# sergcpp/Ray

Hardware: AMD Instinct MI355X
Metric: Msamples/sec (W*H*spp/time) (higher is better)
Workload: dtype f32

## Files before the change

### ray_amd/csrc/rayhip_ctx.hip.h

```cpp
#pragma once

namespace {
thread_local std::string g_err;

int fail(const char *fmt, ...) {
    char buf[1024];
    va_list vl;
    va_start(vl, fmt);
    vsnprintf(buf, sizeof(buf), fmt, vl);
    va_end(vl);
    g_err = buf;
    return 1;
}

#define HIP_TRY(expr)                                                                                                  \
    do {                                                                                                               \
        const hipError_t _e = (expr);                                                                                  \
        if (_e != hipSuccess) {                                                                                        \
            return fail("%s failed: %s (%s:%d)", #expr, hipGetErrorString(_e), __FILE__, __LINE__);                    \
        }                                                                                                              \
    } while (0)

constexpr int MAX_BOUNCE_SLOTS = 130;

// ... 91 lines not shown
    uint32_t cache_path_count = 0;
    DevBuf cache_io;

    int w = 0, h = 0;
    DevBuf px_temp, px_full, px_half, px_raw, px_final, px_base, px_dn, px_req, px_aux_base, px_aux_dn;
    size_t slots_cap = 0;
    DevBuf px_variance, nlm_tm, nlm_var_h, nlm_var;
    DevBuf tonemap_lut;
    DevBuf shard_stage;
    rayhip_update::MeshRefs mesh_refs;
    uint32_t nodes_used = 0, nodes_reserved = 0;
    uint32_t tlas_half = 0;
    int wide = 0;
    uint32_t tex_table[8] = {}, textures_count = 0, tex_flags = 0;
    struct { uint32_t vertices, vtx_indices, tri_materials, materials; } geometry = {};
    bool adaptive_dirty = false;
    int lut_transform = 0, lut_dims = 0;
    PixelBuffers px = {};

    DevBuf ray_planes[2][5], hit_planes[2], shadow_planes[3], deferred_planes[2], point_planes[7], nee_index;
    PointSoA points = {};
    DevBuf pick_plane, record_ray_planes[4];
    RaySoA record_rays = {};
    bool notex_kernels = true;
    bool pick_lds = true;
    bool surface_park = true;
    uint32_t shade_tag = 0;
    uint32_t next_shade_tag() {
        if (++shade_tag == 0u) {
            (void)hipMemsetAsync(pick_plane.p, 0, pick_plane.bytes, stream);
            shade_tag = 1u;
        }
        return shade_tag;
    }
    int shade_split = 29;
    RaySoA rays[2] = {};
    HitSoA hits = {};
    ShadowSoA shadow = {};
    DeferredSoA deferred = {};
    DevBuf counters;
// ... 387 lines not shown
    if (const char *e = getenv("RAYHIP_SORT_KEY")) {
        c->sort_key_mode = std::max(0, std::min(3, atoi(e)));
    }
    if (const char *e = getenv("RAYHIP_SHADE_SPLIT")) {
        c->shade_split = atoi(e) & 31;
        c->shade_form_auto = false;
    }
    if (const char *e = getenv("RAYHIP_NOTEX_KERNELS")) {
        c->notex_kernels = atoi(e) != 0;
    }
    if (const char *e = getenv("RAYHIP_PICK_LDS")) {
        c->pick_lds = atoi(e) != 0;
    }
    if (const char *e = getenv("RAYHIP_SURFACE_PARK")) {
        c->surface_park = atoi(e) != 0;
    }
    {
        const int mode = getenv("RAYHIP_REFILL") != nullptr ? atoi(getenv("RAYHIP_REFILL")) : 3;
        if (mode != 0) {
            int per_cu_refill = 0;
            if (hipOccupancyMaxActiveBlocksPerMultiprocessor(&per_cu_refill, k_trace_closest_refill<8>, WAVE, 0) != hipSuccess || per_cu_refill <= 0) {
                per_cu_refill = per_cu;
            }
            int refill_mult = 16;
            if (const char *e = getenv("RAYHIP_REFILL_MULT")) {
                refill_mult = std::max(1, std::min(64, atoi(e)));
            }
            c->refill_resident = c->props.multiProcessorCount * per_cu_refill;
            {
                int per_cu4 = 0;
// ... 215 lines not shown
```

### ray_amd/csrc/rayhip_render.hip.h

```cpp
#pragma once

static bool pass_fits(const rayhip_ctx *c, const int rect[4], int n) {
    const Layering L = make_layering(c->w, c->h, n);
    const size_t vbytes = size_t(c->w) * size_t(c->h) * size_t(L.cols) * size_t(layer_rows(L)) * 16u;
    return vbytes <= c->px_temp.bytes && (n <= 1 || (vbytes <= c->px_aux_base.bytes && vbytes <= c->px_aux_dn.bytes)) &&
           pass_slots(c, c->w, c->h, rect[2], rect[3], n) + size_t(WAVE) * QUEUE_MAX_STRIPES <= c->slots_cap;
}
static bool rect_inside(const rayhip_ctx *c, const int rect[4]) {
    return rect[0] >= 0 && rect[1] >= 0 && rect[2] > 0 && rect[3] > 0 && rect[0] <= c->w - rect[2] && rect[1] <= c->h - rect[3];
}
static int ensure_pass(rayhip_ctx *c, const int rect[4], int n) {
    if (!rect_inside(c, rect)) {
        return fail("rect outside the frame");
    }
    if (!pass_fits(c, rect, n)) {
        HIP_TRY(hipStreamSynchronize(c->stream));
        if (alloc_frame(c, c->w, c->h, n)) {
            return 1;
        }
    }
    return 0;
}

static void launch_shade(rayhip_ctx *c, const rayhip_camera &cam, int iteration, int bounce, int cur, size_t nslots, uint32_t stripes,
                         int gtrace, int vw, float mix_factor, const Layering &layers, bool plain_ior = false, bool sized = false, int split = -1) {
    ShadeLaunch a;
    a.sc = c->sc;
    a.sp = make_shade_params(cam, iteration, bounce);
    a.sp.plain_ior = plain_ior ? 1u : 0u;
    a.rays_in = c->rays[cur], a.rays_out = c->rays[cur ^ 1];
    a.hits = c->hits, a.shadow = c->shadow, a.deferred = c->deferred, a.points = c->points;
    a.in = c->ray_queue(bounce, nslots, stripes), a.pts = c->point_queue(bounce, nslots, stripes);
    a.out_rays = c->ray_queue(bounce + 1, nslots, stripes), a.out_shadow = c->shadow_queue(bounce, nslots, stripes);
    a.out_deferred = c->deferred_queue(bounce, nslots, stripes), a.nee = c->nee_queue(bounce, nslots, stripes);
    a.out_sky = c->sky_queue(bounce, nslots, stripes), a.sky_index = c->sky_index.as<uint32_t>();
    a.px = c->px, a.layers = layers, a.vw = vw, a.mix_factor = mix_factor;
    a.bounce = bounce, a.grid = gtrace, a.split = split >= 0 ? split : c->shade_split, a.stream = c->stream;
    a.picks = c->pick_plane.as<float4>(), a.record_rays = c->record_rays, a.tag = c->next_shade_tag();
    a.pick_lds = c->pick_lds, a.surface_park = c->surface_park;
    a.no_textures = c->textures_count == 0 && c->notex_kernels;
    if (sized) {
        a.expect[EXPECT_RAYS] = bounce == 0 ? uint32_t(nslots / WAVE + stripes) : c->expect_chunks(bounce, 0, nslots, stripes);
        a.expect[EXPECT_POINTS] = c->expect_chunks(bounce, 3, nslots, stripes), a.expect[EXPECT_LIT] = c->expect_chunks(bounce, 4, nslots, stripes);
        a.expect[EXPECT_DEFERRED] = c->expect_chunks(bounce, 2, nslots, stripes), a.expect[EXPECT_SKY] = c->expect_chunks(bounce, 5, nslots, stripes);
        a.chunks_per_block = c->chunks_per_block;
        a.work = c->next_work(), a.chunks = uint32_t((nslots + WAVE - 1) / WAVE + stripes), a.dyn_mult = c->dyn_mult;
    }
    shade::launch(a);
}

static int render_pass(rayhip_ctx *c, const rayhip_camera *cam, const int rect[4], int iteration, int count_iterations,
                       uint32_t flags, rayhip_stats *stats) {
    if (use_device(c)) {
        return 1;
// ... 346 lines not shown
```

### ray_amd/csrc/rayhip_upload.hip.h

```cpp
#pragma once

static int upload_sky(rayhip_ctx *c, const rayhip_scene_desc *d) {
    c->sky_view = SkyView{};
    if (!(d->env.sky_map_spread_angle > 0.0f) || d->sky_count == 0) {
        return 0;
    }
    if (upload(c, c->sky_desc, d->sky, sizeof(rayhip_sky)) ||
        upload(c, c->sky_transmittance_lut, d->sky_transmittance_lut, size_t(d->sky_transmittance_lut_count) * sizeof(float)) ||
        upload(c, c->sky_multiscatter_lut, d->sky_multiscatter_lut, size_t(d->sky_multiscatter_lut_count) * sizeof(float)) ||
        upload(c, c->sky_dir_lights, d->sky_dir_lights, size_t(d->sky_dir_lights_count) * sizeof(uint32_t)) ||
        upload(c, c->sky_weather, d->sky_weather_tex, d->sky_weather_tex_count) || upload(c, c->sky_noise3d, d->sky_noise3d_tex, d->sky_noise3d_tex_count) ||
        upload(c, c->sky_curl, d->sky_curl_tex, d->sky_curl_tex_count) || upload(c, c->sky_moon, d->sky_moon_tex, d->sky_moon_tex_count) ||
        upload(c, c->sky_cirrus, d->sky_cirrus_tex, d->sky_cirrus_tex_count)) {
        return 1;
    }
    HIP_TRY(hipStreamSynchronize(c->stream));
    SkyView &v = c->sky_view;
    v.desc = c->sky_desc.as<rayhip_sky>();
    v.transmittance_lut = c->sky_transmittance_lut.as<float>(), v.multiscatter_lut = c->sky_multiscatter_lut.as<float>();
    v.dir_lights = c->sky_dir_lights.as<uint32_t>(), v.dir_lights_count = d->sky_dir_lights_count;
    v.weather = c->sky_weather.as<uint8_t>(), v.noise3d = c->sky_noise3d.as<uint8_t>(), v.curl = c->sky_curl.as<uint8_t>();
    v.moon = c->sky_moon.as<uint8_t>(), v.cirrus = c->sky_cirrus.as<uint8_t>();
    return 0;
}
// ... 289 lines not shown
        size_t n_tris = lay.applied ? lay.tris.size() : size_t(d->tris_count);
        rayhip_bvh8::Result b8;
        if (want == 8) {
            b8 = rayhip_bvh8::build(n2, n2_count, mis, d->mesh_instances_count, tlas_root, tris_in, tri_indices_in, uint32_t(n_tris));
            UPLOAD_TRACE(b8.ok ? "bvh8 built" : b8.why_not)
        }
        if (b8.ok && !b8.nodes.empty()) {
            tris_in = b8.tris.data(), tri_indices_in = b8.tri_indices.data(), n_tris = b8.tris.size();
        }
        if (upload(c, c->nodes, n2, size_t(n2_count) * sizeof(rayhip_bvh2_node)) ||
            upload(c, c->tris, tris_in, n_tris * sizeof(rayhip_tri_accel)) ||
            upload(c, c->tri_indices, tri_indices_in, n_tris * sizeof(uint32_t)) ||
            upload(c, c->mesh_instances, mis, size_t(d->mesh_instances_count) * sizeof(rayhip_mesh_instance))) {
            return 1;
        }
        c->tri_pitch = 3;
        if (n_tris && getenv("RAYHIP_TRI_PITCH") && atoi(getenv("RAYHIP_TRI_PITCH")) == 64) {
            DevBuf padded;
            if (padded.alloc(n_tris * 64)) {
                return 1;
            }
            k_pad_tris<<<unsigned((n_tris * 4 + 255) / 256), 256, 0, c->stream>>>(c->tris.as<float4>(), padded.as<float4>(), n_tris);
            HIP_TRY(hipGetLastError());
            HIP_TRY(hipStreamSynchronize(c->stream));
            c->tris.swap(padded);
            padded.release();
            c->tri_pitch = 4;
        }
        size_t wide_bytes = 0;
        if (b8.ok && !b8.nodes.empty()) {
// ... 193 lines not shown
            return 2;
        }
        const uint32_t base = c->nodes_used + c->tlas_half * half;
        c->tlas_half ^= 1u;
        tlas_root = rayhip_update::relocate_top_level(tlas, up, base);
        root_box = tlas.bounds;
        UPLOAD_TRACE("top level built")
        HIP_TRY(hipMemcpyAsync(c->nodes.as<rayhip_bvh2_node>() + base, tlas.nodes.data(), tlas.nodes.size() * sizeof(rayhip_bvh2_node),
                               hipMemcpyHostToDevice, c->stream));
        HIP_TRY(hipStreamSynchronize(c->stream));
    }
    if (upload(c, c->mesh_instances, mis.data(), mis.size() * sizeof(rayhip_mesh_instance)) ||
        (c->wide && upload(c, c->blas_root4, root4.data(), root4.size() * sizeof(uint32_t)))) {
        return 1;
    }
    HIP_TRY(hipStreamSynchronize(c->stream));
    {
        rayhip_scene_desc with_roots = *d;
        if (upload_lights(c, &with_roots) ||
            upload(c, c->env_qtree, d->env_qtree, size_t(d->env_qtree_count) * sizeof(float))) {
            return 1;
        }
    }
    HIP_TRY(hipStreamSynchronize(c->stream));
    if (upload_sky(c, d)) {
        return 1;
    }
    refresh_scene_view(c, d, tlas_root, root_box, uint32_t(live.size()));
    UPLOAD_TRACE("instances updated")
    return 0;
// ... 67 lines not shown
```

### ray_amd/csrc/rt_shade.h

```cpp
#pragma once

#include "rt_sky.h"
#include "shade_lobes.h"

namespace rt {

struct ShadeResult {
    f4 col;
    f3 base_color;
    f4 depth_normal;
    bool emit_secondary, emit_shadow;
    bool defer_sky;
};

RT_HD f3 direct_radiance(const ShadeParams &sp, const Scatter &sct, const f3 throughput) {
    f3 c = sct.direct;
    c *= throughput;
    return clamp_radiance_sum(c, sp.limits[1]);
}
RT_HD float light_pick_random(const SceneView &sc, const ShadeParams &sp, const uint32_t xy, const uint32_t depth) {
    return path_random(sc, sp, xy, depth).get(RAND_DIM_LIGHT_PICK).x;
}
RT_HD LightPick no_light_pick() { return LightPick{0u, 0.0f, 0.0f}; }

RT_HD ShadeResult shade_surface(const SceneView &sc, const ShadeParams &sp, const Hit &hit, const Ray &ray, Ray &new_ray, ShadowRay &sh_r) {
    ShadeResult res;
    res.emit_secondary = res.emit_shadow = false;
    ShadePoint pt;
    SurfaceOut so;
    const bool continues = surface_stage<false>(sc, sp, hit, ray, pt, so);
    res.col = so.radiance;
    res.base_color = so.base_color;
    res.depth_normal = so.normal_depth;
    res.defer_sky = so.deferred_sky;
    if (!continues) {
        return res;
    }
    const LightPick pick = sc.light_cwnodes_count != 0 ? pick_light(sc, pt.P, light_pick_random(sc, sp, ray.xy, ray.depth)) : no_light_pick();
    Scatter sct;
    scatter_stage(sc, sp, ray, pt, pick, sct);
    res.col = mk4(direct_radiance(sp, sct, ray.c), 1.0f);
    res.emit_secondary = sct.has_next, res.emit_shadow = sct.has_shadow;
    new_ray = sct.next, sh_r = sct.shadow;
    return res;
}

}
```

### ray_amd/csrc/shade_kernels.hip

```cpp
#include <hip/hip_runtime.h>

#include <algorithm>
#include <map>
#include <mutex>
#include <utility>

#ifdef RT_PROFILE_SHADE
namespace rt {
__device__ unsigned long long g_prof_shade[64];
}
#define RT_PROF_SHADE_LANES(k)                                                                                          \
    {                                                                                                                   \
        const unsigned long long m_ = __ballot(1);                                                                      \
        if (int(__lane_id()) == __ffsll((long long)m_) - 1) {                                                           \
            atomicAdd(&::rt::g_prof_shade[k], (unsigned long long)__popcll(m_));                                        \
            atomicAdd(&::rt::g_prof_shade[(k) + 1], 1ull);                                                              \
        }                                                                                                               \
    }
#endif

#include "shade_launch.h"

namespace rt {
namespace shade {
// ... 69 lines not shown
            continue;
        }
        const uint32_t i = slot0 + threadIdx.x;
        const bool active = threadIdx.x < n_live;
        bool continues = false, defer = false, sky = false;
        ShadePoint pt;
        SurfaceOut so;
        LightPick pick = no_light_pick();
        if (active) {
            Ray ray = load_ray(rays_in, i, sp.plain_ior == 0u);
            const Hit hit = load_hit(hits, i);
            const uint32_t xy = ray.xy;
            const uint32_t layer = xy_layer(xy, layers);
            const ShadeParams spl = layer_params(sp, layer);
            ray.xy = xy_real(xy, layers, layer);
            continues = surface_stage<true, SKY>(sc, spl, hit, ray, pt, so);
            defer = so.deferred_emitter;
            sky = SKY && so.deferred_sky;
            if (PRIMARY) {
                ShadeResult res;
                res.col = continues ? f4{0.0f, 0.0f, 0.0f, 1.0f} : so.radiance;
                res.base_color = so.base_color, res.depth_normal = so.normal_depth;
                if (layers.count > 1) {
                    write_primary_pixel_layered(res, xy, img_w, px.temp, px.aux_base_layers, px.aux_dn_layers);
                } else {
                    write_primary_pixel(res, xy, img_w, mix_factor, px.temp, px.base_color, px.depth_normals);
                }
            } else if (!continues) {
                ShadeResult res;
                res.col = so.radiance;
                add_secondary_pixel(res, xy, img_w, px.temp);
// ... 156 lines not shown
            }
        }
    }
}

__device__ __forceinline__ uint32_t queue_fill(const RayQueue &q) {
    const uint32_t lane = __lane_id();
    uint32_t n = lane < q.stripes ? q.counts[lane * QUEUE_COUNTER_STRIDE] : 0u;
    for (int m = 32; m >= 1; m >>= 1) {
        n += uint32_t(__shfl_xor(int(n), m));
    }
    return uint32_t(__builtin_amdgcn_readfirstlane(int(n)));
}
__device__ __forceinline__ bool lit_points_are_sparse(const RayQueue &pts, const RayQueue &nee) { return 2u * queue_fill(nee) < queue_fill(pts); }

template <bool NEE, bool CONTINUE, bool INDEXED = false, int MODE = 0>
__global__ void __launch_bounds__(WAVE, (NEE && CONTINUE) ? RT_SCATTER_MIN_WAVES : (NEE ? RT_SCATTER_NEE_MIN_WAVES : RT_SCATTER_CONT_MIN_WAVES)) k_scatter(const SceneView sc, const ShadeParams sp, const RaySoA rays_in,
                                                                       const PointSoA points, const RayQueue in, const RaySoA rays_out,
                                                                       const RayQueue out_rays, const ShadowSoA shadow_out, const RayQueue out_shadow,
                                                                       const PixelBuffers px, const int img_w, const Layering layers,
                                                                       const RayQueue all_points, const RayQueue lit_points) {
    if (MODE != 0 && lit_points_are_sparse(all_points, lit_points) != (MODE == 1)) {
        return;
    }
    const uint32_t n_live_chunks = in.live_chunks();
    ChunkWalk walk(n_live_chunks);
    for (uint32_t c; walk.next(c);) {
        uint32_t stripe, slot0, n_live;
        if (!in.chunk(c, stripe, slot0, n_live)) {
            continue;
        }
        const bool active = threadIdx.x < n_live;
        Scatter sct;
        sct.has_next = sct.has_shadow = false;
        uint32_t xy = 0;
        if (active) {
            uint32_t ray_slot;
            const uint32_t point_slot = INDEXED ? points.nee_index[slot0 + threadIdx.x] : slot0 + threadIdx.x;
            const ShadePoint pt = load_point(points, point_slot, ray_slot);
// ... 1 lines not shown
            Ray ray;
            {
                const float4 d = rays_in.d_cw[ray_slot], cc = rays_in.c_cs[ray_slot];
                const float4 io = sp.plain_ior != 0u ? mkfloat4(-1.0f, -1.0f, -1.0f, -1.0f) : rays_in.ior[ray_slot];
                const uint2 xd = rays_in.xy_depth[ray_slot];
                ray.o = pt.P, ray.pdf = 0.0f;
                ray.d = {d.x, d.y, d.z}, ray.cone_width = d.w;
                ray.c = {cc.x, cc.y, cc.z}, ray.cone_spread = cc.w;
                ray.ior[0] = io.x, ray.ior[1] = io.y, ray.ior[2] = io.z, ray.ior[3] = io.w;
                ray.xy = xd.x, ray.depth = xd.y;
            }
            xy = ray.xy;
            const uint32_t layer = xy_layer(xy, layers);
            const ShadeParams spl = layer_params(sp, layer);
            ray.xy = xy_real(xy, layers, layer);
            scatter_stage<NEE, CONTINUE>(sc, spl, ray, pt, pick, sct);
            sct.next.xy = xy, sct.shadow.xy = xy;
            if (NEE) {
                const f3 col = direct_radiance(spl, sct, ray.c);
                if (col.x != 0.0f || col.y != 0.0f || col.z != 0.0f) {
                    ShadeResult res;
                    res.col = mk4(col, 1.0f);
                    add_secondary_pixel(res, xy, img_w, px.temp);
                }
            }
        }
        if (NEE) {
            const uint32_t sh_slot = out_shadow.alloc(stripe, sct.has_shadow);
            if (sct.has_shadow) {
                store_shadow(shadow_out, sh_slot, sct.shadow);
            }
// ... 109 lines not shown

#ifndef RT_FUSED_NOTEX_MIN_WAVES
#define RT_FUSED_NOTEX_MIN_WAVES 3
#endif
#ifndef RT_FUSED_PARK_MIN_WAVES
#define RT_FUSED_PARK_MIN_WAVES 4
#endif
struct ParkedLane {
    Ray ray;
    float pick[4];
    float pad;
};
constexpr size_t PARK_LDS_BYTES = size_t(WAVE) * sizeof(ParkedLane);
static_assert(sizeof(ParkedLane) % 8u == 4u && PARK_LDS_BYTES <= 10240u, "odd dword stride; at most 10 KB per one-wave block (16 blocks per CU)");
__device__ __forceinline__ void park_fence() { asm volatile("" ::: "memory"); }
template <bool PRIMARY, bool SKY, bool TEX = true, bool PARK = false>
__global__ void __launch_bounds__(WAVE, PARK ? RT_FUSED_PARK_MIN_WAVES : (TEX ? RT_FUSED_MIN_WAVES : RT_FUSED_NOTEX_MIN_WAVES)) k_surface_scatter(const SceneView sc, const ShadeParams sp, const RaySoA rays_in, const HitSoA hits,
                                                                               const RayQueue in, const float4 *__restrict__ picks, const uint32_t tag,
                                                                               const PointSoA records, const RaySoA record_rays, const RayQueue out_records,
                                                                               const RaySoA rays_out, const RayQueue out_rays,
                                                                               const DeferredSoA deferred_out, const RayQueue out_deferred,
                                                                               const PixelBuffers px, const int img_w, const float mix_factor,
                                                                               const Layering layers, uint32_t *__restrict__ sky_index, const RayQueue out_sky) {
    __shared__ ParkedLane s_park[PARK ? WAVE : 1];
    ParkedLane &parked = s_park[PARK ? threadIdx.x : 0u];
    const uint32_t n_live_chunks = in.live_chunks();
    const uint32_t fills = in.fill_counts();
    ChunkWalk walk(n_live_chunks);
    for (uint32_t c; walk.next(c);) {
        uint32_t stripe, slot0, n_live;
        if (!in.chunk(c, fills, stripe, slot0, n_live)) {
            continue;
        }
        const uint32_t i = slot0 + threadIdx.x;
        const bool active = threadIdx.x < n_live;
        bool continues = false, defer = false, sky = false, lit = false;
        ShadePoint pt;
        SurfaceOut so;
        Ray ray_regs;
        Ray &ray = PARK ? parked.ray : ray_regs;
// ... 5 lines not shown
            Ray r = load_ray(rays_in, i, sp.plain_ior == 0u);
            const Hit hit = load_hit(hits, i);
            const float4 pk = picks[i];
            xy = r.xy;
            const uint32_t layer = xy_layer(xy, layers);
            spl = layer_params(sp, layer);
            r.xy = xy_real(xy, layers, layer);
            ahead = vertex_randoms(path_random(sc, spl, r.xy, r.depth));
            if (PARK) {
                parked.ray = r;
                parked.pick[0] = pk.x, parked.pick[1] = pk.y, parked.pick[2] = pk.z, parked.pick[3] = pk.w;
                park_fence();
            } else {
                ray = r, pick = pk;
            }
            continues = surface_stage<true, SKY, TEX>(sc, spl, hit, ray, pt, so, &ahead);
            if (PARK) {
                park_fence();
            }
            defer = so.deferred_emitter;
            sky = SKY && so.deferred_sky;
            if (PRIMARY) {
                ShadeResult res;
                res.col = continues ? f4{0.0f, 0.0f, 0.0f, 1.0f} : so.radiance;
                res.base_color = so.base_color, res.depth_normal = so.normal_depth;
                if (layers.count > 1) {
                    write_primary_pixel_layered(res, xy, img_w, px.temp, px.aux_base_layers, px.aux_dn_layers);
                } else {
                    write_primary_pixel(res, xy, img_w, mix_factor, px.temp, px.base_color, px.depth_normals);
                }
            } else if (!continues) {
// ... 21 lines not shown
            if (sky) {
                sky_index[s_slot] = i;
            }
        }
        if (__any(defer)) {
            const uint32_t d_slot = out_deferred.alloc(stripe, defer);
            if (defer) {
                deferred_out.a[d_slot] = mkfloat4(uint_as_float(i), uint_as_float(so.emitter_triangle), uint_as_float(pt.material), so.emitter_mix_weight);
                deferred_out.b[d_slot] = mkfloat4(pt.base.x, pt.base.y, pt.base.z, 0.0f);
            }
        }
        Scatter sct;
        sct.has_next = sct.has_shadow = false;
        if (continues) {
            ray.o = pt.P, ray.pdf = 0.0f;
            scatter_stage<false, true>(sc, spl, ray, pt, no_light_pick(), sct, &ahead);
            sct.next.xy = xy;
        }
        const uint32_t n_slot = out_rays.alloc(stripe, sct.has_next);
        if (sct.has_next) {
            store_ray(rays_out, n_slot, sct.next, sp.plain_ior == 0u);
        }
    }
}

__global__ void __launch_bounds__(WAVE) k_shade_emissive(const SceneView sc, const ShadeParams sp, const RaySoA rays_in, const HitSoA hits,
                                                        const DeferredSoA deferred, const RayQueue queue, const PixelBuffers px,
                                                        const int img_w) {
    const uint32_t lane = threadIdx.x;
    const uint32_t n_live_chunks = queue.live_chunks();
    ChunkWalk walk(n_live_chunks);
// ... 81 lines not shown
                    const int resident = std::max(1, resident_blocks(reinterpret_cast<const void *>(kernel_wave))) * std::max(1, a.dyn_mult);
                    const uint32_t bound = a.expect[EXPECT_RAYS] != 0u ? a.expect[EXPECT_RAYS] : a.chunks;
                    grid = int(std::max<uint32_t>(1u, std::min<uint32_t>({uint32_t(g), uint32_t(resident), std::max(bound, 1u)})));
                }
                if (lds_nodes != 0u) {
                    kernel<<<(grid + PICK_BLOCK_WAVES - 1) / PICK_BLOCK_WAVES, PICK_BLOCK_WAVES * WAVE, size_t(lds_nodes) * LIGHT_CHILDREN_STRIDE * sizeof(float4), s>>>(
                        a.sc, a.sp, a.rays_in, a.hits, a.in, a.picks, a.tag, a.layers, a.work, lds_nodes);
                } else {
                    kernel_wave<<<grid, WAVE, 0, s>>>(a.sc, a.sp, a.rays_in, a.hits, a.in, a.picks, a.tag, a.layers, a.work, 0u);
                }
            };
            a.work ? go(k_light_pick_first<true, true>, k_light_pick_first<true, false>) : go(k_light_pick_first<false, true>, k_light_pick_first<false, false>);
        }
#define RT_FUSED(...) k_surface_scatter<__VA_ARGS__><<<sized(k_surface_scatter<__VA_ARGS__>, a.expect[EXPECT_RAYS], all), WAVE, 0, s>>>( \
        a.sc, a.sp, a.rays_in, a.hits, a.in, a.picks, a.tag, a.points, a.record_rays, a.nee, a.rays_out, a.out_rays, a.deferred, a.out_deferred, a.px, a.vw, \
        a.mix_factor, a.layers, a.sky_index, a.out_sky)
        const bool sky_scene = a.sc.sky.desc != nullptr, park = a.surface_park;
        if (a.bounce == 0) {
            if (sky_scene) {
                RT_FUSED(true, true);
            } else if (a.no_textures) {
                park ? RT_FUSED(true, false, false, true) : RT_FUSED(true, false, false);
            } else {
                RT_FUSED(true, false);
            }
        } else if (sky_scene) {
            RT_FUSED(false, true);
        } else if (a.no_textures) {
            park ? RT_FUSED(false, false, false, true) : RT_FUSED(false, false, false);
        } else {
            RT_FUSED(false, false);
        }
#undef RT_FUSED
        if (sky_scene) {
            k_shade_sky<<<sized(k_shade_sky, a.expect[EXPECT_SKY], 4096), WAVE, 0, s>>>(a.sc, a.sp, a.rays_in, a.hits, a.sky_index, a.out_sky, a.px, a.vw, a.layers);
        }
        k_shade_emissive<<<sized(k_shade_emissive, a.expect[EXPECT_DEFERRED], 2048), WAVE, 0, s>>>(a.sc, a.sp, a.rays_in, a.hits, a.deferred, a.out_deferred, a.px, a.vw);
        if (lights) {
            k_scatter<true, false><<<sized(k_scatter<true, false>, a.expect[EXPECT_LIT], all), WAVE, 0, s>>>(
                a.sc, a.sp, a.record_rays, a.points, a.nee, a.rays_out, a.out_rays, a.shadow, a.out_shadow, a.px, a.vw, a.layers, a.pts, a.nee);
        }
        return;
    }
    const bool pick_apart = (a.split & 1) != 0 && a.sc.light_cwnodes_count != 0;
#define RT_SURFACE_ARGS a.sc, a.sp, a.rays_in, a.hits, a.in, a.points, a.pts, a.deferred, a.out_deferred, a.px, a.vw, a.mix_factor, a.layers, a.sky_index, a.out_sky
#define RT_SURFACE(...) k_surface<__VA_ARGS__><<<sized(k_surface<__VA_ARGS__>, a.expect[EXPECT_RAYS], all), WAVE, 0, s>>>(RT_SURFACE_ARGS)
    const bool sky = a.sc.sky.desc != nullptr;
    if (a.bounce == 0) {
        if (sky) {
            if (pick_apart) {
                RT_SURFACE(true, false, true);
            } else {
                RT_SURFACE(true, true, true);
            }
        } else if (pick_apart) {
// ... 30 lines not shown
                const uint32_t bound = a.expect[EXPECT_POINTS] != 0u ? a.expect[EXPECT_POINTS] : a.chunks;
                grid = int(std::max<uint32_t>(1u, std::min<uint32_t>({uint32_t(g), uint32_t(resident), std::max(bound, 1u)})));
            }
            kernel<<<grid, WAVE, 0, s>>>(a.sc, a.sp, a.rays_in, a.points, a.pts, a.nee, a.layers, a.work);
        };
        if (a.work) {
            nee_compact ? go(k_light_pick_refill<true, true>) : go(k_light_pick_refill<false, true>);
        } else {
            nee_compact ? go(k_light_pick_refill<true, false>) : go(k_light_pick_refill<false, false>);
        }
    } else if (nee_compact) {
        k_light_pick<true><<<sized(k_light_pick<true>, a.expect[EXPECT_POINTS], all), WAVE, 0, s>>>(a.sc, a.sp, a.rays_in, a.points, a.pts, a.nee, a.layers);
    } else if (pick_apart) {
        k_light_pick<false><<<sized(k_light_pick<false>, a.expect[EXPECT_POINTS], all), WAVE, 0, s>>>(a.sc, a.sp, a.rays_in, a.points, a.pts, a.nee, a.layers);
    }
#define RT_SCATTER_ARGS(queue) a.sc, a.sp, a.rays_in, a.points, queue, a.rays_out, a.out_rays, a.shadow, a.out_shadow, a.px, a.vw, a.layers, a.pts, a.nee
#define RT_SCATTER(queue, expect, ...) k_scatter<__VA_ARGS__><<<sized(k_scatter<__VA_ARGS__>, expect, all), WAVE, 0, s>>>(RT_SCATTER_ARGS(queue))
    if (nee_compact) {
        RT_SCATTER(a.nee, a.expect[EXPECT_LIT], true, false, true, 1);
        RT_SCATTER(a.pts, a.expect[EXPECT_POINTS], false, true, false, 1);
        RT_SCATTER(a.pts, a.expect[EXPECT_POINTS], true, true, false, 2);
    } else if ((a.split & 2) != 0) {
        RT_SCATTER(a.pts, a.expect[EXPECT_POINTS], true, false);
        RT_SCATTER(a.pts, a.expect[EXPECT_POINTS], false, true);
    } else {
        RT_SCATTER(a.pts, a.expect[EXPECT_POINTS], true, true);
    }
#undef RT_SCATTER
#undef RT_SCATTER_ARGS
}

// ... 16 lines not shown
```

### ray_amd/csrc/shade_launch.h

```cpp
#pragma once

#include "rt_shade.h"
#include "wavefront.hip.h"

namespace rt {

struct PointSoA {
    float4 *p_slot;
    float4 *n_gx;
    float4 *b_gy;
    float4 *base_gz;
    float4 *scalars;
    float4 *misc;
    float4 *light;
    uint32_t *nee_index;
};

struct ShadeLaunch {
    SceneView sc;
    ShadeParams sp;
    RaySoA rays_in, rays_out;
    HitSoA hits;
    ShadowSoA shadow;
    DeferredSoA deferred;
// ... 1 lines not shown
    RayQueue in, pts, out_rays, out_shadow, out_deferred, nee, out_sky;
    uint32_t *sky_index;
    PixelBuffers px;
    Layering layers;
    int vw;
    float mix_factor;
    int bounce, grid;
    uint32_t expect[5] = {0, 0, 0, 0, 0};
    int chunks_per_block = 0;
    uint32_t *work = nullptr;
    uint32_t chunks = 0;
    int dyn_mult = 1;
    bool no_textures = false;
    bool pick_lds = true;
    bool surface_park = true;
    float4 *picks = nullptr;
    uint32_t tag = 0;
    RaySoA record_rays = {};
    int split;
    hipStream_t stream;
};
enum { EXPECT_RAYS = 0, EXPECT_POINTS, EXPECT_LIT, EXPECT_DEFERRED, EXPECT_SKY };
namespace shade {
void launch(const ShadeLaunch &a);
}

}
```

### ray_amd/csrc/shade_lobes.h

```cpp
#pragma once

#include "shade_point.h"

namespace rt {

struct Scatter {
    f3 direct;
    Ray next;
    ShadowRay shadow;
    bool has_next, has_shadow;
};

struct ScatterFrame {
    f3 P, T, B, N, Ng;
    f3 I;
    f3 wo;
    float floor_alpha;
    float mix_weight;
    bool mis;
};
RT_HD f3 to_tangent(const ScatterFrame &fr, const f3 v) { return tangent_from_world(fr.T, fr.B, fr.N, v); }
RT_HD f3 to_world(const ScatterFrame &fr, const f3 v) { return world_from_tangent(fr.T, fr.B, fr.N, v); }

RT_HD float nee_mis_weight(const ScatterFrame &fr, const LightSample &ls, const float bsdf_pdf) {
// ... 313 lines not shown
                next.cone_spread += MAX_CONE_SPREAD_INCREMENT * fminf(L.transmit_alpha.x, L.transmit_alpha.y);
                if (!pt.backfacing) {
                    ior_stack_enter(next.ior, L.inside_ior);
                } else {
                    ior_stack_leave(next.ior);
                }
            }
            const float pdf = v.pdf * L.p_transmit;
            scale_throughput(next, v.f, safe_div_pos(fr.mix_weight, pdf));
            next.pdf = pdf;
            next.d = dir;
        }
    }
}

template <bool NEE = true, bool CONTINUE = true>
RT_HD void scatter_stage(const SceneView &sc, const ShadeParams &sp, const Ray &ray, const ShadePoint &pt, const LightPick &pick, Scatter &out,
                         const VertexRandoms *ahead = nullptr) {
    RT_PROF_SHADE_LANES(0)
    const PassLimits &ps = sp.ps;
    const rayhip_material &mat = sc.materials[pt.material];
    const PathRandom rnd = path_random(sc, sp, ray.xy, ray.depth);

    ScatterFrame fr;
    fr.P = pt.P, fr.N = pt.N, fr.B = pt.B, fr.Ng = pt.plane_N;
    fr.T = tangent_of(pt);
    fr.I = ray.d;
    fr.wo = to_tangent(fr, -fr.I);
    fr.floor_alpha = (get_diff_depth(ray.depth) > 0) ? ps.regularize_alpha : 0.0f;
    fr.mix_weight = pt.mix_weight;
    const int n_diff = get_diff_depth(ray.depth), n_spec = get_spec_depth(ray.depth), n_refr = get_refr_depth(ray.depth);
    const int n_total = n_diff + n_spec + n_refr;
    fr.mis = n_total < ps.max_total_depth;

    LightSample ls = no_light_sample();
    if (NEE && sc.light_cwnodes_count != 0) {
// ... 83 lines not shown
```

### ray_amd/csrc/shade_point.h

```cpp
#pragma once

#include "shade_lights.h"
#include "shade_math.h"

namespace rt {

struct PassLimits {
    int max_diff_depth, max_spec_depth, max_refr_depth, max_transp_depth, max_total_depth;
    int min_total_depth, min_transp_depth;
    float regularize_alpha;
};
struct ShadeParams {
    PassLimits ps;
    float limits[2];
    uint32_t rand_seed;
    int iteration;
    uint32_t plain_ior;
};

struct PathRandom {
    uint32_t hash, dim;
    int sample;
    const uint32_t *table;
    RT_HD f2 get(const int which) const { return get_scrambled_2d_rand(dim + uint32_t(which), hash, sample, table); }
// ... 175 lines not shown
    }
    float nee_pdf = solid_angle_triangle(transform_point(origin, inst->inv_xform), p1, p2, p3, f2{0.0f, 0.0f}, nullptr) / inv_pick_prob;
    if (nee_pdf == 0.0f) {
        nee_pdf = (t * t) / (0.5f * twice_area * cos_theta * inv_pick_prob);
    }
    return power_heuristic(bsdf_pdf, nee_pdf);
}
RT_HD f4 emissive_hit_radiance(const ShadeParams &sp, const float mix_weight, const float mis_weight, const float strength, const f3 base,
                               const f3 throughput) {
    f3 c = {0.0f, 0.0f, 0.0f};
    c += mix_weight * mis_weight * strength * base;
    c *= throughput;
    return mk4(clamp_radiance_sum(c, sp.limits[1]), 1.0f);
}

template <bool DEFER_EMITTERS, bool SKY = true, bool TEX = true>
RT_HD bool surface_stage(const SceneView &sc, const ShadeParams &sp, const Hit &hit, const Ray &ray, ShadePoint &pt, SurfaceOut &out,
                         const VertexRandoms *ahead = nullptr) {
    out.radiance = f4{0.0f, 0.0f, 0.0f, 0.0f};
    out.base_color = f3{0.0f, 0.0f, 0.0f};
    out.normal_depth = f4{0.0f, 0.0f, 0.0f, 0.0f};
    out.deferred_emitter = false;
    out.deferred_sky = false;

    const PathRandom rnd = path_random(sc, sp, ray.xy, ray.depth);
    struct {
        const PathRandom &rnd;
        bool have;
        f2 v;
        RT_HD f2 operator()() {
            if (!have) {
                v = rnd.get(RAND_DIM_TEX), have = true;
// ... 16 lines not shown
        }
        out.radiance = c;
        return false;
    }
    if (hit.obj_index < 0) {
        f3 c = emitter_radiance(sc, ray, hit, tex_jitter);
        c *= ray.c;
        out.radiance = mk4(clamp_radiance_sum(c, sp.limits[0]), 1.0f);
        return false;
    }

    const f3 view = ray.d;
    pt.P = ray.o + hit.t * view;
    pt.backfacing = (hit.prim_index < 0);
    const uint32_t tri = pt.backfacing ? uint32_t(-hit.prim_index - 1) : uint32_t(hit.prim_index);
    const rayhip_mesh_instance *inst = &sc.mesh_instances[hit.obj_index];
    const float4 *rows = sc.tri_verts + size_t(tri) * TRI_VERTS_STRIDE;
    const Corner c1 = load_corner(rows), c2 = load_corner(rows + 2), c3 = load_corner(rows + 4);
    const float4 plane = rows[6];
    const float4 row7 = rows[7];
    const float uv_area = row7.x;
    const rayhip_tri_mat_data sides = {uint16_t(float_as_uint(row7.y) & 0xffffu), uint16_t(float_as_uint(row7.y) >> 16)};

    const float w1 = 1.0f - hit.u - hit.v;
    const f3 N_obj = normalize(c1.n * w1 + c2.n * hit.u + c3.n * hit.v);
    const f2 uv = c1.uv * w1 + c2.uv * hit.u + c3.uv * hit.v;
    const float twice_area_obj = plane.w;
    f3 Ng = {plane.x, plane.y, plane.z}, N = N_obj;

    const rayhip_material *mat = &sc.materials[sides.front_mi & MATERIAL_INDEX_BITS];
    if (pt.backfacing) {
        if (sides.back_mi == 0xffff) {
            return false;
        }
        mat = &sc.materials[sides.back_mi & MATERIAL_INDEX_BITS];
        Ng = -Ng, N = -N;
    }
    Ng = safe_normalize(transform_normal(Ng, inst->inv_xform));
    N = safe_normalize(transform_normal(N, inst->inv_xform));

    pt.cone_width = ray.cone_width + ray.cone_spread * hit.t;
    float lod_lambda = 0.5f * fast_log2(uv_area / twice_area_obj);
    lod_lambda += fast_log2(pt.cone_width);

    const float outside_ior = peek_ior_stack(ray.ior, pt.backfacing);

    const f2 pick = ahead ? ahead->bsdf_pick : rnd.get(RAND_DIM_BSDF_PICK);
    float mix_u = pick.x;
    pt.mix_weight = 1.0f;
    while (mat->type == NODE_MIX) {
        float k = mat->tangent_rotation_or_strength;
        if (TEX && mat->textures[BASE_TEXTURE] != 0xffffffff) {
            k *= sample_color(sc, mat->textures[BASE_TEXTURE], uv, 0, tex_jitter()).x;
        }
        const float eta = pt.backfacing ? safe_div_pos(outside_ior, mat->ior) : safe_div_pos(mat->ior, outside_ior);
        const float fresnel = mat->ior != 0.0f ? fresnel_dielectric(dot(view, N), eta) : 1.0f;
        k *= saturatef(fresnel);
        const bool additive = (mat->flags & MAT_FLAG_MIX_ADD) != 0;
        if (mix_u > k) {
            pt.mix_weight *= additive ? 1.0f / (1.0f - k) : 1.0f;
            mat = &sc.materials[mat->textures[MIX_MAT1]];
            mix_u = safe_div_pos(mix_u - k, 1.0f - k);
        } else {
            pt.mix_weight *= additive ? 1.0f / k : 1.0f;
            mat = &sc.materials[mat->textures[MIX_MAT2]];
            mix_u = safe_div_pos(mix_u, k);
        }
    }
    pt.mix_pick = mix_u;
    pt.material = uint32_t(mat - sc.materials);

    if (TEX && mat->textures[NORMALS_TEXTURE] != 0xffffffff) {
        f4 nm = sample_bilinear(sc, mat->textures[NORMALS_TEXTURE], uv, 0, tex_jitter());
        nm = nm * 2.0f;
        nm = {nm.x - 1.0f, nm.y - 1.0f, nm.z - 1.0f, nm.w - 1.0f};
        nm.z = 1.0f;
        if (mat->textures[NORMALS_TEXTURE] & TEX_RECONSTRUCT_Z_BIT) {
            nm.z = safe_sqrt(1.0f - nm.x * nm.x - nm.y * nm.y);
        }
        const float4 *brow = sc.tri_bitangents + size_t(tri) * TRI_BITANGENTS_STRIDE;
        const float4 b1 = brow[0], b2 = brow[1], b3 = brow[2];
        f3 Bt = f3{b1.x, b1.y, b1.z} * w1 + f3{b2.x, b2.y, b2.z} * hit.u + f3{b3.x, b3.y, b3.z} * hit.v;
        f3 Tg = cross(Bt, N_obj);
        if (pt.backfacing) {
            Bt = -Bt, Tg = -Tg;
        }
        Bt = safe_normalize(transform_normal(Bt, inst->inv_xform));
        Tg = safe_normalize(transform_normal(Tg, inst->inv_xform));
        const f3 smooth = N;
        N = normalize(nm.x * Tg + nm.z * N + nm.y * Bt);
        if (mat->normal_map_strength_unorm != 0xffff) {
            N = normalize(smooth + (N - smooth) * (float(mat->normal_map_strength_unorm) / 65535.0f));
        }
        N = keep_reflection_above_surface(Ng, -view, N);
    }

    const f3 P_obj = c1.p * w1 + c2.p * hit.u + c3.p * hit.v;
    f3 radial = transform_normal(f3{-P_obj.z, 0.0f, P_obj.x}, inst->inv_xform);
    if (length2(cross(radial, N)) == 0.0f) {
        radial = transform_normal(P_obj, inst->inv_xform);
    }
    if (mat->tangent_rotation_or_strength != 0.0f) {
        radial = rotate_about_axis(radial, N, mat->tangent_rotation_or_strength);
    }
    pt.N = N;
    pt.plane_N = Ng;
    pt.B = safe_normalize(cross(radial, N));

    pt.base = mk3(mat->base_color);
    if (TEX && mat->textures[BASE_TEXTURE] != 0xffffffff) {
        const uint32_t tex = mat->textures[BASE_TEXTURE];
        pt.base *= xyz(sample_color(sc, tex, uv, int(get_texture_lod(sc, tex, lod_lambda)), tex_jitter()));
    }
    out.base_color = pt.base;
    out.normal_depth = mk4(N, hit.t);
// ... 25 lines not shown
            pt.specular *= s.x;
        }
    }

    if (mat->type != NODE_EMISSIVE) {
        return true;
    }
    float mis = 1.0f;
    if ((ray.depth & 0x00ffffff) != 0 && (mat->flags & MAT_FLAG_IMP_SAMPLE)) {
        if (DEFER_EMITTERS) {
            out.deferred_emitter = true;
            out.emitter_triangle = tri;
            out.emitter_mix_weight = pt.mix_weight;
            mis = 0.0f;
        } else {
            mis = emissive_hit_mis_weight(sc, ray.o, view, pt.P, hit.t, ray.pdf, tri, inst);
        }
    }
    out.radiance = emissive_hit_radiance(sp, pt.mix_weight, mis, mat->tangent_rotation_or_strength, pt.base, ray.c);
    return false;
}

}
```

Before: 743.1.

## Stage material and instance transform tables in LDS for untextured shade kernels

```diff
diff --git a/ray_amd/csrc/rayhip_ctx.hip.h b/ray_amd/csrc/rayhip_ctx.hip.h
--- a/ray_amd/csrc/rayhip_ctx.hip.h
+++ b/ray_amd/csrc/rayhip_ctx.hip.h
@@ -129,6 +129,7 @@
     int wide = 0;
     uint32_t tex_table[8] = {}, textures_count = 0, tex_flags = 0;
     struct { uint32_t vertices, vtx_indices, tri_materials, materials; } geometry = {};
+    uint32_t instances_count = 0;
     bool adaptive_dirty = false;
     int lut_transform = 0, lut_dims = 0;
     PixelBuffers px = {};
@@ -139,6 +140,8 @@
     RaySoA record_rays = {};
     bool notex_kernels = true;
     bool pick_lds = true;
+    bool shade_lds_tables = true;
+    uint32_t shade_lds_materials_max = 0xffffffffu, shade_lds_instances_max = 0xffffffffu;
     bool surface_park = true;
     uint32_t shade_tag = 0;
     uint32_t next_shade_tag() {
@@ -556,6 +559,15 @@
     }
     if (const char *e = getenv("RAYHIP_SURFACE_PARK")) {
         c->surface_park = atoi(e) != 0;
+    }
+    if (const char *e = getenv("RAYHIP_SHADE_LDS_TABLES")) {
+        c->shade_lds_tables = atoi(e) != 0;
+    }
+    if (const char *e = getenv("RAYHIP_SHADE_LDS_MATERIALS_MAX")) {
+        c->shade_lds_materials_max = uint32_t(std::max(0, atoi(e)));
+    }
+    if (const char *e = getenv("RAYHIP_SHADE_LDS_INSTANCES_MAX")) {
+        c->shade_lds_instances_max = uint32_t(std::max(0, atoi(e)));
     }
     {
         const int mode = getenv("RAYHIP_REFILL") != nullptr ? atoi(getenv("RAYHIP_REFILL")) : 3;
diff --git a/ray_amd/csrc/rayhip_render.hip.h b/ray_amd/csrc/rayhip_render.hip.h
--- a/ray_amd/csrc/rayhip_render.hip.h
+++ b/ray_amd/csrc/rayhip_render.hip.h
@@ -38,6 +38,8 @@
     a.bounce = bounce, a.grid = gtrace, a.split = split >= 0 ? split : c->shade_split, a.stream = c->stream;
     a.picks = c->pick_plane.as<float4>(), a.record_rays = c->record_rays, a.tag = c->next_shade_tag();
     a.pick_lds = c->pick_lds, a.surface_park = c->surface_park;
+    a.lds_tables = c->shade_lds_tables, a.n_materials = c->geometry.materials, a.n_instances = c->instances_count;
+    a.lds_materials_max = c->shade_lds_materials_max, a.lds_instances_max = c->shade_lds_instances_max;
     a.no_textures = c->textures_count == 0 && c->notex_kernels;
     if (sized) {
         a.expect[EXPECT_RAYS] = bounce == 0 ? uint32_t(nslots / WAVE + stripes) : c->expect_chunks(bounce, 0, nslots, stripes);
diff --git a/ray_amd/csrc/rayhip_upload.hip.h b/ray_amd/csrc/rayhip_upload.hip.h
--- a/ray_amd/csrc/rayhip_upload.hip.h
+++ b/ray_amd/csrc/rayhip_upload.hip.h
@@ -327,6 +327,7 @@
             upload(c, c->mesh_instances, mis, size_t(d->mesh_instances_count) * sizeof(rayhip_mesh_instance))) {
             return 1;
         }
+        c->instances_count = d->mesh_instances_count;
         c->tri_pitch = 3;
         if (n_tris && getenv("RAYHIP_TRI_PITCH") && atoi(getenv("RAYHIP_TRI_PITCH")) == 64) {
             DevBuf padded;
@@ -550,6 +551,7 @@
         (c->wide && upload(c, c->blas_root4, root4.data(), root4.size() * sizeof(uint32_t)))) {
         return 1;
     }
+    c->instances_count = uint32_t(mis.size());
     HIP_TRY(hipStreamSynchronize(c->stream));
     {
         rayhip_scene_desc with_roots = *d;
diff --git a/ray_amd/csrc/rt_shade.h b/ray_amd/csrc/rt_shade.h
--- a/ray_amd/csrc/rt_shade.h
+++ b/ray_amd/csrc/rt_shade.h
@@ -28,7 +28,7 @@
     res.emit_secondary = res.emit_shadow = false;
     ShadePoint pt;
     SurfaceOut so;
-    const bool continues = surface_stage<false>(sc, sp, hit, ray, pt, so);
+    const bool continues = surface_stage<false>(sc, scene_tables(sc), sp, hit, ray, pt, so);
     res.col = so.radiance;
     res.base_color = so.base_color;
     res.depth_normal = so.normal_depth;
@@ -38,7 +38,7 @@
     }
     const LightPick pick = sc.light_cwnodes_count != 0 ? pick_light(sc, pt.P, light_pick_random(sc, sp, ray.xy, ray.depth)) : no_light_pick();
     Scatter sct;
-    scatter_stage(sc, sp, ray, pt, pick, sct);
+    scatter_stage(sc, scene_tables(sc), sp, ray, pt, pick, sct);
     res.col = mk4(direct_radiance(sp, sct, ray.c), 1.0f);
     res.emit_secondary = sct.has_next, res.emit_shadow = sct.has_shadow;
     new_ray = sct.next, sh_r = sct.shadow;
diff --git a/ray_amd/csrc/shade_kernels.hip b/ray_amd/csrc/shade_kernels.hip
--- a/ray_amd/csrc/shade_kernels.hip
+++ b/ray_amd/csrc/shade_kernels.hip
@@ -107,7 +107,7 @@
             const uint32_t layer = xy_layer(xy, layers);
             const ShadeParams spl = layer_params(sp, layer);
             ray.xy = xy_real(xy, layers, layer);
-            continues = surface_stage<true, SKY>(sc, spl, hit, ray, pt, so);
+            continues = surface_stage<true, SKY>(sc, scene_tables(sc), spl, hit, ray, pt, so);
             defer = so.deferred_emitter;
             sky = SKY && so.deferred_sky;
             if (PRIMARY) {
@@ -294,15 +294,51 @@
 }
 __device__ __forceinline__ bool lit_points_are_sparse(const RayQueue &pts, const RayQueue &nee) { return 2u * queue_fill(nee) < queue_fill(pts); }
 
-template <bool NEE, bool CONTINUE, bool INDEXED = false, int MODE = 0>
+constexpr uint32_t LDS_MATERIALS_MAX = 48, LDS_INSTANCES_MAX = 14;
+constexpr uint32_t MATERIAL_WORDS = uint32_t(sizeof(rayhip_material) / 4u), INV_XFORM_WORDS = 12;
+constexpr uint32_t LDS_TABLE_WORDS = LDS_MATERIALS_MAX * MATERIAL_WORDS + LDS_INSTANCES_MAX * INV_XFORM_WORDS;
+constexpr size_t LDS_TABLE_BYTES = size_t(LDS_TABLE_WORDS) * 4u;
+static_assert(sizeof(rayhip_material) % 4u == 0u && alignof(rayhip_material) <= 4u, "the material table is copied and addressed as dwords");
+struct LdsTables {
+    const uint32_t *words;
+    __device__ __forceinline__ const rayhip_material &material(const uint32_t i) const { return reinterpret_cast<const rayhip_material *>(words)[i]; }
+    __device__ __forceinline__ const float *inv_xform(const uint32_t i) const {
+        return reinterpret_cast<const float *>(words) + LDS_MATERIALS_MAX * MATERIAL_WORDS + i * INV_XFORM_WORDS;
+    }
+};
+__device__ __forceinline__ void fill_lds_tables(uint32_t *words, const SceneView &sc, const uint32_t n_materials, const uint32_t n_instances) {
+    const uint32_t *src = reinterpret_cast<const uint32_t *>(sc.materials);
+    for (uint32_t r = threadIdx.x; r < n_materials * MATERIAL_WORDS; r += blockDim.x) {
+        words[r] = src[r];
+    }
+    for (uint32_t r = threadIdx.x; r < n_instances * INV_XFORM_WORDS; r += blockDim.x) {
+        words[LDS_MATERIALS_MAX * MATERIAL_WORDS + r] = float_as_uint(sc.mesh_instances[r / INV_XFORM_WORDS].inv_xform[r % INV_XFORM_WORDS]);
+    }
+    __syncthreads();
+}
+template <bool LDS_TABLES>
+__device__ __forceinline__ auto stage_tables(const SceneView &sc, const uint32_t *words) {
+    if constexpr (LDS_TABLES) {
+        return LdsTables{words};
+    } else {
+        return scene_tables(sc);
+    }
+}
+
+template <bool NEE, bool CONTINUE, bool INDEXED = false, int MODE = 0, bool LDS_TABLES = false>
 __global__ void __launch_bounds__(WAVE, (NEE && CONTINUE) ? RT_SCATTER_MIN_WAVES : (NEE ? RT_SCATTER_NEE_MIN_WAVES : RT_SCATTER_CONT_MIN_WAVES)) k_scatter(const SceneView sc, const ShadeParams sp, const RaySoA rays_in,
                                                                        const PointSoA points, const RayQueue in, const RaySoA rays_out,
                                                                        const RayQueue out_rays, const ShadowSoA shadow_out, const RayQueue out_shadow,
                                                                        const PixelBuffers px, const int img_w, const Layering layers,
-                                                                       const RayQueue all_points, const RayQueue lit_points) {
+                                                                       const RayQueue all_points, const RayQueue lit_points, const uint32_t n_materials) {
     if (MODE != 0 && lit_points_are_sparse(all_points, lit_points) != (MODE == 1)) {
         return;
     }
+    __shared__ uint32_t s_tables[LDS_TABLES ? LDS_TABLE_WORDS : 1];
+    if (LDS_TABLES) {
+        fill_lds_tables(s_tables, sc, n_materials, 0u);
+    }
+    const auto tb = stage_tables<LDS_TABLES>(sc, s_tables);
     const uint32_t n_live_chunks = in.live_chunks();
     ChunkWalk walk(n_live_chunks);
     for (uint32_t c; walk.next(c);) {
@@ -334,7 +370,7 @@
             const uint32_t layer = xy_layer(xy, layers);
             const ShadeParams spl = layer_params(sp, layer);
             ray.xy = xy_real(xy, layers, layer);
-            scatter_stage<NEE, CONTINUE>(sc, spl, ray, pt, pick, sct);
+            scatter_stage<NEE, CONTINUE>(sc, tb, spl, ray, pt, pick, sct);
             sct.next.xy = xy, sct.shadow.xy = xy;
             if (NEE) {
                 const f3 col = direct_radiance(spl, sct, ray.c);
@@ -474,16 +510,23 @@
 constexpr size_t PARK_LDS_BYTES = size_t(WAVE) * sizeof(ParkedLane);
 static_assert(sizeof(ParkedLane) % 8u == 4u && PARK_LDS_BYTES <= 10240u, "odd dword stride; at most 10 KB per one-wave block (16 blocks per CU)");
 __device__ __forceinline__ void park_fence() { asm volatile("" ::: "memory"); }
-template <bool PRIMARY, bool SKY, bool TEX = true, bool PARK = false>
+static_assert(PARK_LDS_BYTES + LDS_TABLE_BYTES <= 10240u, "parked slots + tables: at most 10 KB per one-wave block (16 blocks per CU)");
+template <bool PRIMARY, bool SKY, bool TEX = true, bool PARK = false, bool LDS_TABLES = false>
 __global__ void __launch_bounds__(WAVE, PARK ? RT_FUSED_PARK_MIN_WAVES : (TEX ? RT_FUSED_MIN_WAVES : RT_FUSED_NOTEX_MIN_WAVES)) k_surface_scatter(const SceneView sc, const ShadeParams sp, const RaySoA rays_in, const HitSoA hits,
                                                                                const RayQueue in, const float4 *__restrict__ picks, const uint32_t tag,
                                                                                const PointSoA records, const RaySoA record_rays, const RayQueue out_records,
                                                                                const RaySoA rays_out, const RayQueue out_rays,
                                                                                const DeferredSoA deferred_out, const RayQueue out_deferred,
                                                                                const PixelBuffers px, const int img_w, const float mix_factor,
-                                                                               const Layering layers, uint32_t *__restrict__ sky_index, const RayQueue out_sky) {
+                                                                               const Layering layers, uint32_t *__restrict__ sky_index, const RayQueue out_sky,
+                                                                               const uint32_t n_materials, const uint32_t n_instances) {
     __shared__ ParkedLane s_park[PARK ? WAVE : 1];
+    __shared__ uint32_t s_tables[LDS_TABLES ? LDS_TABLE_WORDS : 1];
     ParkedLane &parked = s_park[PARK ? threadIdx.x : 0u];
+    if (LDS_TABLES) {
+        fill_lds_tables(s_tables, sc, n_materials, n_instances);
+    }
+    const auto tb = stage_tables<LDS_TABLES>(sc, s_tables);
     const uint32_t n_live_chunks = in.live_chunks();
     const uint32_t fills = in.fill_counts();
     ChunkWalk walk(n_live_chunks);
@@ -519,7 +562,7 @@
             } else {
                 ray = r, pick = pk;
             }
-            continues = surface_stage<true, SKY, TEX>(sc, spl, hit, ray, pt, so, &ahead);
+            continues = surface_stage<true, SKY, TEX>(sc, tb, spl, hit, ray, pt, so, &ahead);
             if (PARK) {
                 park_fence();
             }
@@ -571,7 +614,7 @@
         sct.has_next = sct.has_shadow = false;
         if (continues) {
             ray.o = pt.P, ray.pdf = 0.0f;
-            scatter_stage<false, true>(sc, spl, ray, pt, no_light_pick(), sct, &ahead);
+            scatter_stage<false, true>(sc, tb, spl, ray, pt, no_light_pick(), sct, &ahead);
             sct.next.xy = xy;
         }
         const uint32_t n_slot = out_rays.alloc(stripe, sct.has_next);
@@ -683,20 +726,30 @@
         }
 #define RT_FUSED(...) k_surface_scatter<__VA_ARGS__><<<sized(k_surface_scatter<__VA_ARGS__>, a.expect[EXPECT_RAYS], all), WAVE, 0, s>>>( \
         a.sc, a.sp, a.rays_in, a.hits, a.in, a.picks, a.tag, a.points, a.record_rays, a.nee, a.rays_out, a.out_rays, a.deferred, a.out_deferred, a.px, a.vw, \
-        a.mix_factor, a.layers, a.sky_index, a.out_sky)
+        a.mix_factor, a.layers, a.sky_index, a.out_sky, a.n_materials, a.n_instances)
         const bool sky_scene = a.sc.sky.desc != nullptr, park = a.surface_park;
+        const bool lds_tables = a.lds_tables && a.n_materials != 0u && a.n_materials <= std::min(a.lds_materials_max, LDS_MATERIALS_MAX) &&
+                                a.n_instances != 0u && a.n_instances <= std::min(a.lds_instances_max, LDS_INSTANCES_MAX);
         if (a.bounce == 0) {
             if (sky_scene) {
                 RT_FUSED(true, true);
             } else if (a.no_textures) {
-                park ? RT_FUSED(true, false, false, true) : RT_FUSED(true, false, false);
+                if (lds_tables) {
+                    park ? RT_FUSED(true, false, false, true, true) : RT_FUSED(true, false, false, false, true);
+                } else {
+                    park ? RT_FUSED(true, false, false, true) : RT_FUSED(true, false, false);
+                }
             } else {
                 RT_FUSED(true, false);
             }
         } else if (sky_scene) {
             RT_FUSED(false, true);
         } else if (a.no_textures) {
-            park ? RT_FUSED(false, false, false, true) : RT_FUSED(false, false, false);
+            if (lds_tables) {
+                park ? RT_FUSED(false, false, false, true, true) : RT_FUSED(false, false, false, false, true);
+            } else {
+                park ? RT_FUSED(false, false, false, true) : RT_FUSED(false, false, false);
+            }
         } else {
             RT_FUSED(false, false);
         }
@@ -706,8 +759,11 @@
         }
         k_shade_emissive<<<sized(k_shade_emissive, a.expect[EXPECT_DEFERRED], 2048), WAVE, 0, s>>>(a.sc, a.sp, a.rays_in, a.hits, a.deferred, a.out_deferred, a.px, a.vw);
         if (lights) {
-            k_scatter<true, false><<<sized(k_scatter<true, false>, a.expect[EXPECT_LIT], all), WAVE, 0, s>>>(
-                a.sc, a.sp, a.record_rays, a.points, a.nee, a.rays_out, a.out_rays, a.shadow, a.out_shadow, a.px, a.vw, a.layers, a.pts, a.nee);
+            auto nee = [&](auto kernel) {
+                kernel<<<sized(kernel, a.expect[EXPECT_LIT], all), WAVE, 0, s>>>(
+                    a.sc, a.sp, a.record_rays, a.points, a.nee, a.rays_out, a.out_rays, a.shadow, a.out_shadow, a.px, a.vw, a.layers, a.pts, a.nee, a.n_materials);
+            };
+            (lds_tables && a.no_textures) ? nee(k_scatter<true, false, false, 0, true>) : nee(k_scatter<true, false>);
         }
         return;
     }
@@ -768,7 +824,7 @@
     } else if (pick_apart) {
         k_light_pick<false><<<sized(k_light_pick<false>, a.expect[EXPECT_POINTS], all), WAVE, 0, s>>>(a.sc, a.sp, a.rays_in, a.points, a.pts, a.nee, a.layers);
     }
-#define RT_SCATTER_ARGS(queue) a.sc, a.sp, a.rays_in, a.points, queue, a.rays_out, a.out_rays, a.shadow, a.out_shadow, a.px, a.vw, a.layers, a.pts, a.nee
+#define RT_SCATTER_ARGS(queue) a.sc, a.sp, a.rays_in, a.points, queue, a.rays_out, a.out_rays, a.shadow, a.out_shadow, a.px, a.vw, a.layers, a.pts, a.nee, a.n_materials
 #define RT_SCATTER(queue, expect, ...) k_scatter<__VA_ARGS__><<<sized(k_scatter<__VA_ARGS__>, expect, all), WAVE, 0, s>>>(RT_SCATTER_ARGS(queue))
     if (nee_compact) {
         RT_SCATTER(a.nee, a.expect[EXPECT_LIT], true, false, true, 1);
diff --git a/ray_amd/csrc/shade_launch.h b/ray_amd/csrc/shade_launch.h
--- a/ray_amd/csrc/shade_launch.h
+++ b/ray_amd/csrc/shade_launch.h
@@ -39,6 +39,9 @@
     bool no_textures = false;
     bool pick_lds = true;
     bool surface_park = true;
+    bool lds_tables = true;
+    uint32_t n_materials = 0, n_instances = 0;
+    uint32_t lds_materials_max = 0xffffffffu, lds_instances_max = 0xffffffffu;
     float4 *picks = nullptr;
     uint32_t tag = 0;
     RaySoA record_rays = {};
diff --git a/ray_amd/csrc/shade_lobes.h b/ray_amd/csrc/shade_lobes.h
--- a/ray_amd/csrc/shade_lobes.h
+++ b/ray_amd/csrc/shade_lobes.h
@@ -351,12 +351,12 @@
     }
 }
 
-template <bool NEE = true, bool CONTINUE = true>
-RT_HD void scatter_stage(const SceneView &sc, const ShadeParams &sp, const Ray &ray, const ShadePoint &pt, const LightPick &pick, Scatter &out,
+template <bool NEE = true, bool CONTINUE = true, class Tables = SceneTables>
+RT_HD void scatter_stage(const SceneView &sc, const Tables &tb, const ShadeParams &sp, const Ray &ray, const ShadePoint &pt, const LightPick &pick, Scatter &out,
                          const VertexRandoms *ahead = nullptr) {
     RT_PROF_SHADE_LANES(0)
     const PassLimits &ps = sp.ps;
-    const rayhip_material &mat = sc.materials[pt.material];
+    const rayhip_material &mat = tb.material(pt.material);
     const PathRandom rnd = path_random(sc, sp, ray.xy, ray.depth);
 
     ScatterFrame fr;
diff --git a/ray_amd/csrc/shade_point.h b/ray_amd/csrc/shade_point.h
--- a/ray_amd/csrc/shade_point.h
+++ b/ray_amd/csrc/shade_point.h
@@ -213,8 +213,16 @@
     return mk4(clamp_radiance_sum(c, sp.limits[1]), 1.0f);
 }
 
-template <bool DEFER_EMITTERS, bool SKY = true, bool TEX = true>
-RT_HD bool surface_stage(const SceneView &sc, const ShadeParams &sp, const Hit &hit, const Ray &ray, ShadePoint &pt, SurfaceOut &out,
+struct SceneTables {
+    const rayhip_material *materials;
+    const rayhip_mesh_instance *instances;
+    RT_HD const rayhip_material &material(const uint32_t i) const { return materials[i]; }
+    RT_HD const float *inv_xform(const uint32_t i) const { return instances[i].inv_xform; }
+};
+RT_HD SceneTables scene_tables(const SceneView &sc) { return SceneTables{sc.materials, sc.mesh_instances}; }
+
+template <bool DEFER_EMITTERS, bool SKY = true, bool TEX = true, class Tables = SceneTables>
+RT_HD bool surface_stage(const SceneView &sc, const Tables &tb, const ShadeParams &sp, const Hit &hit, const Ray &ray, ShadePoint &pt, SurfaceOut &out,
                          const VertexRandoms *ahead = nullptr) {
     out.radiance = f4{0.0f, 0.0f, 0.0f, 0.0f};
     out.base_color = f3{0.0f, 0.0f, 0.0f};
@@ -261,7 +269,7 @@
     pt.P = ray.o + hit.t * view;
     pt.backfacing = (hit.prim_index < 0);
     const uint32_t tri = pt.backfacing ? uint32_t(-hit.prim_index - 1) : uint32_t(hit.prim_index);
-    const rayhip_mesh_instance *inst = &sc.mesh_instances[hit.obj_index];
+    const float *inv_xform = tb.inv_xform(uint32_t(hit.obj_index));
     const float4 *rows = sc.tri_verts + size_t(tri) * TRI_VERTS_STRIDE;
     const Corner c1 = load_corner(rows), c2 = load_corner(rows + 2), c3 = load_corner(rows + 4);
     const float4 plane = rows[6];
@@ -275,16 +283,16 @@
     const float twice_area_obj = plane.w;
     f3 Ng = {plane.x, plane.y, plane.z}, N = N_obj;
 
-    const rayhip_material *mat = &sc.materials[sides.front_mi & MATERIAL_INDEX_BITS];
+    uint32_t mat_index = sides.front_mi & MATERIAL_INDEX_BITS;
     if (pt.backfacing) {
         if (sides.back_mi == 0xffff) {
             return false;
         }
-        mat = &sc.materials[sides.back_mi & MATERIAL_INDEX_BITS];
+        mat_index = sides.back_mi & MATERIAL_INDEX_BITS;
         Ng = -Ng, N = -N;
     }
-    Ng = safe_normalize(transform_normal(Ng, inst->inv_xform));
-    N = safe_normalize(transform_normal(N, inst->inv_xform));
+    Ng = safe_normalize(transform_normal(Ng, inv_xform));
+    N = safe_normalize(transform_normal(N, inv_xform));
 
     pt.cone_width = ray.cone_width + ray.cone_spread * hit.t;
     float lod_lambda = 0.5f * fast_log2(uv_area / twice_area_obj);
@@ -295,6 +303,7 @@
     const f2 pick = ahead ? ahead->bsdf_pick : rnd.get(RAND_DIM_BSDF_PICK);
     float mix_u = pick.x;
     pt.mix_weight = 1.0f;
+    const rayhip_material *mat = &tb.material(mat_index);
     while (mat->type == NODE_MIX) {
         float k = mat->tangent_rotation_or_strength;
         if (TEX && mat->textures[BASE_TEXTURE] != 0xffffffff) {
@@ -306,16 +315,17 @@
         const bool additive = (mat->flags & MAT_FLAG_MIX_ADD) != 0;
         if (mix_u > k) {
             pt.mix_weight *= additive ? 1.0f / (1.0f - k) : 1.0f;
-            mat = &sc.materials[mat->textures[MIX_MAT1]];
+            mat_index = mat->textures[MIX_MAT1];
             mix_u = safe_div_pos(mix_u - k, 1.0f - k);
         } else {
             pt.mix_weight *= additive ? 1.0f / k : 1.0f;
-            mat = &sc.materials[mat->textures[MIX_MAT2]];
+            mat_index = mat->textures[MIX_MAT2];
             mix_u = safe_div_pos(mix_u, k);
         }
+        mat = &tb.material(mat_index);
     }
     pt.mix_pick = mix_u;
-    pt.material = uint32_t(mat - sc.materials);
+    pt.material = mat_index;
 
     if (TEX && mat->textures[NORMALS_TEXTURE] != 0xffffffff) {
         f4 nm = sample_bilinear(sc, mat->textures[NORMALS_TEXTURE], uv, 0, tex_jitter());
@@ -332,8 +342,8 @@
         if (pt.backfacing) {
             Bt = -Bt, Tg = -Tg;
         }
-        Bt = safe_normalize(transform_normal(Bt, inst->inv_xform));
-        Tg = safe_normalize(transform_normal(Tg, inst->inv_xform));
+        Bt = safe_normalize(transform_normal(Bt, inv_xform));
+        Tg = safe_normalize(transform_normal(Tg, inv_xform));
         const f3 smooth = N;
         N = normalize(nm.x * Tg + nm.z * N + nm.y * Bt);
         if (mat->normal_map_strength_unorm != 0xffff) {
@@ -343,9 +353,9 @@
     }
 
     const f3 P_obj = c1.p * w1 + c2.p * hit.u + c3.p * hit.v;
-    f3 radial = transform_normal(f3{-P_obj.z, 0.0f, P_obj.x}, inst->inv_xform);
+    f3 radial = transform_normal(f3{-P_obj.z, 0.0f, P_obj.x}, inv_xform);
     if (length2(cross(radial, N)) == 0.0f) {
-        radial = transform_normal(P_obj, inst->inv_xform);
+        radial = transform_normal(P_obj, inv_xform);
     }
     if (mat->tangent_rotation_or_strength != 0.0f) {
         radial = rotate_about_axis(radial, N, mat->tangent_rotation_or_strength);
@@ -401,7 +411,7 @@
             out.emitter_mix_weight = pt.mix_weight;
             mis = 0.0f;
         } else {
-            mis = emissive_hit_mis_weight(sc, ray.o, view, pt.P, hit.t, ray.pdf, tri, inst);
+            mis = emissive_hit_mis_weight(sc, ray.o, view, pt.P, hit.t, ray.pdf, tri, &sc.mesh_instances[hit.obj_index]);
         }
     }
     out.radiance = emissive_hit_radiance(sp, pt.mix_weight, mis, mat->tangent_rotation_or_strength, pt.base, ray.c);
```

Measured after the change: 762.4 (median of 6 runs). 1.03x the previous value.
